# Xinglab/abPOA

Hardware: AMD Instinct MI355X
Metric: read-sets/sec (consensus bit-exact) + DP Gcells/sec (roofline.dp_gcells_per_s) (higher is better)
Workload: dtype int16

## Files before the change

### abpoa_amd/csrc/msa_device.cpp

```cpp
#include <algorithm>
#include <atomic>
#include <chrono>
#include <limits.h>
#include <mutex>
#include <stdio.h>
#include <stdlib.h>
#include <string.h>
#include <thread>
#include <vector>
#include <hip/hip_runtime.h>
#include "engine_options.h"
#include "batch_stream.h"
#include "msa_device.h"
#include "poa_device.h"
#include "poa_graph.h"
#include "dir_plane.h"
#include "msa_batch.h"
#include "msa_device_debug.h"
#include "msa_device_plan.h"

namespace abpoa_hip {

namespace {
#define HIP_OK(expr, code) do { hipError_t e_ = (expr); if (e_ != hipSuccess) { \
// ... 242 lines not shown
    p.nd_base = dg + L.o_base; p.nd_nin = dg + L.o_nin; p.nd_nout = dg + L.o_nout; p.nd_naln = dg + L.o_naln;
    p.nd_in = (int32_t *)(dg + L.o_in); p.nd_out = (int32_t *)(dg + L.o_out); p.nd_outw = (int32_t *)(dg + L.o_outw); p.nd_aln = (int32_t *)(dg + L.o_aln);
    p.nd_inx = (int32_t *)(dg + L.o_inx); p.nd_outx = (int32_t *)(dg + L.o_outx); p.nd_outwx = (int32_t *)(dg + L.o_outwx);
    p.nd_nread = (int32_t *)(dg + L.o_nread); p.nd_row = (int32_t *)(dg + L.o_row);
    p.t_out = (int32_t *)(dg + L.o_tout); p.t_outw = (int32_t *)(dg + L.o_toutw); p.t_in = (int32_t *)(dg + L.o_tin);
    p.nd_rid = (uint64_t *)(dg + L.o_rid); p.msa_rank = (int32_t *)(dg + L.o_mrank); p.msa_off = (const int64_t *)(dg + L.o_msaoff); p.msa_out = nullptr;
    p.row_node[0] = (int32_t *)(dg + L.o_order0); p.row_node[1] = (int32_t *)(dg + L.o_order1);
    p.scratch = (int32_t *)(dr + L.o_scratch);
    p.aln = (AlnDesc *)(dr + L.o_aln_desc); p.out = (AlnOut *)(dr + L.o_out_rec);
    p.row_base = dr + L.o_rbase; p.row_sdist = dr + L.o_rsd; p.row_pd = (uint32_t *)(dr + L.o_rpd); p.row_node_id = (int32_t *)(dr + L.o_rnid);
    p.row_remain = (int32_t *)(dr + L.o_rrem);
    p.pred_off = (int32_t *)(dr + L.o_poff); p.pred_row = (int32_t *)(dr + L.o_pred); p.cigar = (uint64_t *)(dr + L.o_cigar);
    p.out_off = gen_io ? (int32_t *)(dr + L.o_ooff) : nullptr; p.out_row = gen_io ? (int32_t *)(dr + L.o_orow) : nullptr;
    if (pl.amb) {
        p.reads_rc = di + L.o_rc; p.wts_rc = J.any_w ? (int32_t *)(di + L.o_wrc) : nullptr; p.is_rc = dg + L.o_isrc; p.retry = dr + L.o_retry;
        p.out_fwd = (AlnOut *)(dr + L.o_outfwd); p.cigar_fwd = (uint64_t *)(dr + L.o_cigfwd);
    }
    p.cons_node = (int32_t *)(dg + L.o_cnode); p.cons_cov = (int32_t *)(dg + L.o_ccov); p.cons_base = dg + L.o_cbase;
}

int final_lds_plan(const Job &J, DevBatch &b) {
    const DevicePlan &pl = J.pl; const abpoa_hip_scoring_t *sc = &pl.sc;
    int32_t inf_dummy; const int max_bits = abpoa_hip_score_bits(sc, pl.max_node_cap, pl.max_qlen, &inf_dummy); const int pn = max_bits == 16 ? 16 : 8;
    const int64_t width = padded_width(pl.max_qlen, pn);
    const int64_t est_plain = pl.est_cols(width, pl.w_max, pn), est_ragged = std::min<int64_t>(std::max<int64_t>(est_plain, std::min<int64_t>(1024, width)),
            est_plain + pl.max_extra);
    make_lds_plan(sc, pl.max_qlen, max_bits, est_ragged, J.n_sets, &b.lds);
    if (pl.max_extra > 0 && b.lds.fr_cols == 0) make_lds_plan(sc, pl.max_qlen, max_bits, est_plain, J.n_sets, &b.lds);
    if (pl.general) { b.lds.wide_on = 0; b.lds.fr_cols = 0; b.lds.loc_cols = 0; }
    else if (pl.local) {
        b.lds.wide_on = 0;
        if (max_bits != 16 || b.lds.loc_cols <= 0 || (pl.max_qlen / 16 + 1) * 16 > b.lds.loc_cols || pl.max_qlen > b.lds.q_cap) {
                set_err("local alignment outside the device row loop's range"); return ABPOA_HIP_EINVAL; }
    }
    int min_qlen = pl.max_qlen;
    for (int s = 0; s < J.n_sets; ++s) for (int r = 1; r < J.sets[s].n_reads; ++r) min_qlen = std::min(min_qlen, J.sets[s].lens[r]);
    const int min_bits = abpoa_hip_score_bits(sc, 3, min_qlen, &inf_dummy);
    b.bits_mask = (min_bits == 16 ? 1 : 0) | (max_bits == 32 ? 2 : 0);
    const int w_min = std::min(sc->wb + (int)(sc->wf * (float)min_qlen), pl.max_extra ? pl.weff_lo : INT_MAX), w_top = std::max(pl.w_max, pl.weff_hi);
    const bool mixed = pl.max_extra > 0;
    if (!mixed && (w_top < b.lds.wide_w_lo || w_min > b.lds.wide_w_hi)) b.lds.wide_on = 0;
    b.lds.narrow_off = (!mixed && b.lds.wide_on >= 1 && w_min >= b.lds.wide_w_lo && w_top <= b.lds.wide_w_hi) ? 1 : 0;
    return 0;
}

int fill_dev_batch(Job &J, bool *want_general) {
    const DevicePlan &pl = J.pl; Cache &C = *J.C; const Layout &L = J.L; const abpoa_hip_scoring_t *sc = &pl.sc; const PoaDev &p = J.p; DevBatch &b = J.b, &b_rc = J.b_rc;
    uint8_t *di = C.in.dev, *dr = C.rows.dev; const bool gen_io = pl.gen_io(); int rc;
    memset(&b, 0, sizeof(b));
    b.n = J.n_sets; b.m = sc->m;
    if ((rc = final_lds_plan(J, b))) return rc;
    if (!pl.local && !pl.general && (b.lds.fr_cols == 0 || pl.max_qlen > b.lds.q_cap)) { *want_general = true; set_err("band too wide for the fast row loop"); return ABPOA_HIP_EINVAL; }
    b.o1 = sc->gap_open1; b.e1 = sc->gap_ext1; b.o2 = sc->gap_open2; b.e2 = sc->gap_ext2;
    b.align_mode = sc->align_mode; b.gap_mode = sc->gap_mode; b.wb = sc->wb; b.zdrop = sc->zdrop; b.ret_cigar = 1; b.rev_cigar = 0;
    b.want_trace = 0; b.fresh_band = 1; b.want_lr = 0;
    b.dbg = opt_int("ABPOA_HIP_DBG", 0);
    b.mat = (const int32_t *)(di + L.o_mat); b.aln = p.aln; b.out = p.out;
    b.dir_mode = pl.dir ? (pl.dir_wide ? 2 : 1) : 0; b.row_sdist = p.row_sdist; b.row_pd = p.row_pd;
    b.query = p.reads; b.row_base = p.row_base; b.row_node_id = p.row_node_id; b.row_remain = p.row_remain; b.row_active = p.row_base;
    b.pred_off = p.pred_off; b.pred_row = p.pred_row; b.out_off = p.pred_off; b.out_row = p.pred_row;
    b.left = p.scratch; b.right = p.scratch;
    if (gen_io) {
        b.out_off = p.out_off; b.out_row = p.out_row; b.left = (int32_t *)(dr + L.o_left); b.right = (int32_t *)(dr + L.o_right); b.row_active = dr + L.o_act;
    }
    b.dp_beg_sn = (int32_t *)(dr + L.o_bsn); b.dp_end_sn = (int32_t *)(dr + L.o_esn); b.row_cell_off = (int64_t *)(dr + L.o_coff);
    b.row_max_i = (int32_t *)(dr + L.o_rmi);
    b.planes = C.planes.dev; b.cigar = p.cigar;
    b_rc = b;
    if (pl.amb) {
        b.want_lr = (sc->wb >= 0 && !pl.general) ? 1 : 0;
        b_rc = b; b_rc.want_lr = 0; b_rc.fresh_band = sc->wb >= 0 ? 0 : 1;
    }
    return 0;
}

void plan_rounds(Job &J) {
    const DevicePlan &pl = J.pl; const abpoa_hip_scoring_t *sc = &pl.sc; const PoaDev &p = J.p; const DevBatch &b = J.b; DevBatch &b_r = J.b_r;
    bool &dbg_sync = J.dbg_sync, &use_rounds = J.use_rounds; size_t &rounds_lds = J.rounds_lds;
    dbg_sync = opt_on("ABPOA_HIP_DEVSYNC");
    use_rounds = !pl.local && pl.rounds_possible && !dbg_sync && b.lds.wide_on == 0 && !(b.dbg & 64) && pl.max_reads > 2 && !opt_on("ABPOA_HIP_LOCKSTEP");
    b_r = b; rounds_lds = 0;
    if (use_rounds) {
        auto dyn_of = [&](const DevBatch &x) { return std::max<size_t>(std::max<size_t>((size_t)x.lds.total_rows, (size_t)x.lds.total_tail),
                std::max<size_t>((size_t)5 * (size_t)(p.lds_rows > 0 ? p.lds_rows : 0), (size_t)16 * 256)); };
        rounds_lds = dyn_of(b_r);
        int st_lds = 0; int nb = poa_rounds_residency(sc->gap_mode, rounds_lds, &st_lds);
        if (nb < 4 && J.n_sets > nb * 256) {
            const int budget = 160 * 1024 / 4 - st_lds - 512, excess = (int)rounds_lds - budget;
            if (excess > 0 && (size_t)b_r.lds.total_tail == rounds_lds && b_r.lds.bt_bytes_tail - ((excess + 15) & ~15) >= 8 * 1024) {
                b_r.lds.bt_bytes_tail -= (excess + 15) & ~15; b_r.lds.total_tail -= (excess + 15) & ~15;
                rounds_lds = dyn_of(b_r); nb = poa_rounds_residency(sc->gap_mode, rounds_lds, &st_lds);
            }
        }
        b_r.lds.te_on = 0;
        if (b_r.dir_mode && sc->gap_mode != ABPOA_HIP_LINEAR_GAP && !opt_on("ABPOA_HIP_LATE_TAIL")) {
            const int avail = (int)rounds_lds - b_r.lds.phase_off, tables = (SPEC_WK - 1) * SPEC_PM_ROWS * 4;
            const int ring = (b_r.lds.total_rows - b_r.lds.phase_off + 15) & ~15;
            int w_ = ((avail - tables) / SPEC_WK) & ~15, m_ = w_;
            if (w_ < ring) { m_ = ring; w_ = ((avail - tables - m_) / (SPEC_WK - 1)) & ~15; }
            if (w_ >= SPEC_EARLY_MIN) { b_r.lds.te_on = 1; b_r.lds.te_main = m_; b_r.lds.te_w = w_; }
        }
        const int n_cu = device_cu_count(J.device);
        if (nb < 1 || J.n_sets > nb * n_cu) use_rounds = false;
        if (opt_set("ABPOA_HIP_VERBOSE")) fprintf(stderr,
                "[abpoa-hip] all-rounds kernel: %s, %zu B dynamic + %d B static LDS per workgroup, %d workgroups per CU, " "backtrack window %d B, helpers %s (%d + 3 x %d B)\n",
                use_rounds ? "on" : "off", rounds_lds, st_lds, nb, b_r.lds.bt_bytes_tail, b_r.lds.te_on ? "under the row loop" : "after the row loop", b_r.lds.te_main, b_r.lds.te_w);
    }
}

int queue_job(Job &J, DeviceDebug &dbg) {
    const DevicePlan &pl = J.pl; Cache &C = *J.C; const Layout &L = J.L; PoaDev &p = J.p; const DevBatch &b = J.b;
    hipStream_t st = C.stream; uint8_t *hi = C.in.host, *hg = C.graph.host, *dg = C.graph.dev, *dr = C.rows.dev; int rc;
    const int64_t *roff = (const int64_t *)(hi + L.o_roff);
    auto stage = [&](const char *what, int k) { return dbg.stage(what, k); };
    if (pl.gen_io()) HIP_OK(hipMemsetAsync(dr + L.o_act, 1, (size_t)pl.node_tot, st), ABPOA_HIP_ELAUNCH);
    if (pl.amb) HIP_OK(hipMemsetAsync(dg + L.o_isrc, 0, (size_t)pl.tot_reads, st), ABPOA_HIP_ELAUNCH);
    J.t_queue = now_s();
    HIP_OK(hipEventRecord(C.ev[0], st), ABPOA_HIP_ELAUNCH);
    if (stage("upload", 0)) return ABPOA_HIP_ELAUNCH;
    HIP_OK(launch_poa_init(p, st), ABPOA_HIP_ELAUNCH);
    if (stage("init", 0)) return ABPOA_HIP_ELAUNCH;
    dbg.graph_check(0);
    HIP_OK(hipEventRecord(C.ev[1], st), ABPOA_HIP_ELAUNCH);
    for (int k = 1; k < pl.max_reads; ++k) {
        if (k == 2 && !J.rest_up) {
            stage_reads(J, 2, pl.max_reads);
            HIP_OK(hipMemcpyAsync(C.in.dev + L.o_reads + (size_t)J.split_at, hi + L.o_reads + (size_t)J.split_at, (size_t)(roff[pl.tot_reads] - J.split_at),
                    hipMemcpyHostToDevice, C.copy_stream), ABPOA_HIP_ELAUNCH);
            HIP_OK(hipEventRecord(C.ev_copy, C.copy_stream), ABPOA_HIP_ELAUNCH);
            HIP_OK(hipStreamWaitEvent(st, C.ev_copy, 0), ABPOA_HIP_ELAUNCH);
            J.rest_up = true;
        }
        if (J.use_rounds && k == 2) {
            HIP_OK(hipEventRecord(C.ev[2], st), ABPOA_HIP_ELAUNCH);
            HIP_OK(launch_poa_rounds(p, J.b_r, (int32_t *)(dr + L.o_ticket), C.in.host + L.o_rargs, J.slot, 2, J.rounds_lds, st), ABPOA_HIP_ELAUNCH);
            HIP_OK(hipEventRecord(C.ev[3], st), ABPOA_HIP_ELAUNCH);
            break;
        }
        p.round = k;
        hipEvent_t *e = C.ev.data() + 4 * k;
        if (p.order_mode) { HIP_OK(launch_poa_order(p, st), ABPOA_HIP_ELAUNCH); if (stage("row order", k)) return ABPOA_HIP_ELAUNCH; dbg.order_check(k); }
        HIP_OK(launch_poa_prepare(p, st), ABPOA_HIP_ELAUNCH);
        if (stage("prepare", k)) return ABPOA_HIP_ELAUNCH;
        HIP_OK(hipEventRecord(e[0], st), ABPOA_HIP_ELAUNCH);
        if (pl.general) { HIP_OK(launch_dp_general(b, st), ABPOA_HIP_ELAUNCH); HIP_OK(hipEventRecord(e[1], st), ABPOA_HIP_ELAUNCH); }
        else HIP_OK(launch_dp_fast(b, st, e[1]), ABPOA_HIP_ELAUNCH);
        if (stage("dp rows + tail", k)) return ABPOA_HIP_ELAUNCH;
        if (pl.amb) {
            HIP_OK(launch_poa_strand_check(p, st), ABPOA_HIP_ELAUNCH);
            HIP_OK(launch_dp_general(J.b_rc, st), ABPOA_HIP_ELAUNCH);
            HIP_OK(launch_poa_strand_pick(p, st), ABPOA_HIP_ELAUNCH);
            if (stage("strand retry", k)) return ABPOA_HIP_ELAUNCH;
        }
        dbg.balance_report(k, b, e[0], e[1]);
        HIP_OK(hipEventRecord(e[2], st), ABPOA_HIP_ELAUNCH);
        HIP_OK(launch_poa_fuse(p, st), ABPOA_HIP_ELAUNCH);
        if (stage("fuse", k)) return ABPOA_HIP_ELAUNCH;
        dbg.graph_check(k);
        HIP_OK(hipEventRecord(e[3], st), ABPOA_HIP_ELAUNCH);
    }
    if (pl.want_cons) { HIP_OK(launch_poa_consensus(p, st), ABPOA_HIP_ELAUNCH); if (stage("consensus", pl.max_reads)) return ABPOA_HIP_ELAUNCH; }
    if (pl.want_msa) { HIP_OK(launch_poa_msa_rank(p, st), ABPOA_HIP_ELAUNCH); if (stage("msa rank", pl.max_reads)) return ABPOA_HIP_ELAUNCH; }
    HIP_OK(hipMemcpyAsync(hg, dg, J.dl_bytes, hipMemcpyDeviceToHost, st), ABPOA_HIP_ELAUNCH);
    HIP_OK(hipStreamSynchronize(st), ABPOA_HIP_ELAUNCH);
    int64_t msa_total = 0;
    if (pl.want_msa) {
        const PoaState *hs_ = (const PoaState *)(hg + L.o_state);
// ... 173 lines not shown
```

### abpoa_amd/csrc/poa_bodies.h

```cpp
#pragma once
#include <hip/hip_runtime.h>
#include <stdint.h>
#include <limits.h>
#include <string.h>
#include "poa_device.h"
#include "../../include/abpoa_hip.h"

namespace abpoa_hip {

namespace {

__device__ __forceinline__ int imin_(int a, int b) { return a < b ? a : b; }
__device__ __forceinline__ int imax_(int a, int b) { return a > b ? a : b; }
__device__ __forceinline__ int ld_fresh(const int32_t *p) { return __hip_atomic_load(p, __ATOMIC_RELAXED, __HIP_MEMORY_SCOPE_AGENT); }
constexpr int POA_TERM_MAX = 250;
__device__ __forceinline__ int32_t &in_slot(const PoaDev &p, const PoaSet &S, int64_t X, int t) {
    return t < POA_HOT ? p.nd_in[X * POA_HOT + t] : (t < p.in_cap ? p.nd_inx[X * (p.in_cap - POA_HOT) + t - POA_HOT] : p.t_in[S.term0 + t - p.in_cap]);
}
__device__ __forceinline__ int32_t &out_slot(const PoaDev &p, const PoaSet &S, int64_t X, int t) {
    return t < POA_HOT ? p.nd_out[X * POA_HOT + t] : (t < p.out_cap ? p.nd_outx[X * (p.out_cap - POA_HOT) + t - POA_HOT] : p.t_out[S.term0 + t - p.out_cap]);
}
__device__ __forceinline__ int32_t &outw_slot(const PoaDev &p, const PoaSet &S, int64_t X, int t) {
    return t < POA_HOT ? p.nd_outw[X * POA_HOT + t] : (t < p.out_cap ? p.nd_outwx[X * (p.out_cap - POA_HOT) + t - POA_HOT] : p.t_outw[S.term0 + t - p.out_cap]);
}
// ... 162 lines not shown
        const int incl = wave_scan_add(np);
        if (lane == 63) wtot[wave] = incl;
        __syncthreads();
        int before = 0, all = 0;
#pragma unroll
        for (int w_ = 0; w_ < GW; ++w_) { const int x_ = wtot[w_]; all += x_; before += w_ < wave ? x_ : 0; }
        const int off = carry + before + incl - np;
        if (r < n) p.pred_off[N0 + r] = off;
        if (off + np > S.pred_cap) overflow = true;
        carry += all;
        __syncthreads();
    }
    {
        for (int r0 = tid; r0 < n; r0 += 4 * GT) {
            int u[4], np[4], off[4]; int4 i4[4];
#pragma unroll
            for (int j = 0; j < 4; ++j) { const int r = r0 + j * GT; const bool ok = r < n; u[j] = order[ok ? r : 0]; off[j] = p.pred_off[N0 + (ok ? r : 0)];
                                          np[j] = !ok ? 0 : (in_lds ? (int)np_lds[r] : (r > 0 ? (int)p.nd_nin[N0 + u[j]] : 0)); }
#pragma unroll
            for (int j = 0; j < 4; ++j) { if (off[j] + np[j] > S.pred_cap) np[j] = 0; i4[j] = *(const int4 *)(p.nd_in + (N0 + u[j]) * POA_HOT); }
            int pr[4][4];
#pragma unroll
            for (int j = 0; j < 4; ++j) {
                pr[j][0] = np[j] > 0 ? p.nd_row[N0 + i4[j].x] : 0; pr[j][1] = np[j] > 1 ? p.nd_row[N0 + i4[j].y] : 0;
                pr[j][2] = np[j] > 2 ? p.nd_row[N0 + i4[j].z] : 0; pr[j][3] = np[j] > 3 ? p.nd_row[N0 + i4[j].w] : 0;
            }
#pragma unroll
            for (int j = 0; j < 4; ++j) {
                int32_t *dst = p.pred_row + S.pred0 + off[j];
                const int r = r0 + j * GT;
                unsigned long long pdv = ~0ull;
#pragma unroll
                for (int t = 0; t < 4; ++t) {
                    if (t < np[j]) { dst[t] = pr[j][t]; if (r - pr[j][t] <= 254) pdv = (pdv & ~(0xffull << (8 * t))) | ((unsigned long long)(r - pr[j][t]) << (8 * t)); }
                }
                for (int t = POA_HOT; t < np[j]; ++t) { const int pr_ = p.nd_row[N0 + in_slot(p, S, N0 + u[j], t)]; dst[t] = pr_;
                        if (t < 8 && r - pr_ <= 254) pdv = (pdv & ~(0xffull << (8 * t))) | ((unsigned long long)(r - pr_) << (8 * t)); }
                if (r < n) { p.row_pd[2 * (N0 + r)] = (unsigned)pdv; p.row_pd[2 * (N0 + r) + 1] = (unsigned)(pdv >> 32); }
            }
        }
    }
    if (tid == 0) p.pred_off[N0 + n] = carry;
    if (p.out_off) {
        int carry_o = 0;
        for (int t0 = 0; t0 < n; t0 += GT) {
            const int r = t0 + tid;
            const int u = r < n ? order[r] : 0;
            const int no = r < n ? (int)p.nd_nout[N0 + u] : 0;
            const int incl = wave_scan_add(no);
            __syncthreads();
            if (lane == 63) wtot[wave] = incl;
            __syncthreads();
            int before = 0, all = 0;
#pragma unroll
            for (int w_ = 0; w_ < GW; ++w_) { const int x_ = wtot[w_]; all += x_; before += w_ < wave ? x_ : 0; }
            const int off = carry_o + before + incl - no;
            if (r < n) {
                p.out_off[N0 + r] = off;
                if (off + no > S.pred_cap) overflow = true;
                else for (int t = 0; t < no; ++t) p.out_row[S.pred0 + off + t] = p.nd_row[N0 + out_slot(p, S, N0 + u, t)];
            }
            carry_o += all;
        }
        if (tid == 0) p.out_off[N0 + n] = carry_o;
    }
    overflow = __syncthreads_or(overflow);
    if (tid == 0) {
        AlnDesc d; memset(&d, 0, sizeof(d));
        const int qlen = p.read_len[S.read0 + k];
        d.n_rows = n; d.qlen = qlen;
        d.bits = score_bits(p, n, qlen, &d.inf_min);
        d.w = p.wb < 0 ? qlen : p.wb + (int)(p.wf * (float)qlen);
        d.cigar_cap = S.cigar_cap; d.flags = (p.general & 1) ? 0 : ALN_FAST_OK; d.pad0 = S.band_extra;
        d.query_off = p.read_off[S.read0 + k]; d.row0 = N0; d.poff0 = N0; d.pred0 = S.pred0; d.out0 = S.pred0;
        d.plane_off = S.plane_off; d.plane_cap = S.plane_cap / (d.bits / 8); d.cigar_off = S.cigar_off;
        if (overflow || n + qlen + 8 > S.cigar_cap) { st->status = POA_ST_FALLBACK; st->reason = overflow ? POA_WHY_PRED_SLOTS : POA_WHY_CIGAR_SLOTS; d.flags = ALN_SKIP; d.n_rows = 3; }
        p.aln[s] = d;
        p.out[s].status = 0; p.out[s].n_cigar = 0; p.out[s].n_cells = 0;
    }
}

__device__ __forceinline__ void poa_fuse_body(const PoaDev &p, const int s, const int k) {
    const int tid = threadIdx.x, lane = tid & 63, wave = tid >> 6;
    __shared__ int sh_fail, sh_nodes, wtot[GW];
    const PoaSet S = p.sets[s];
    PoaState *st = p.state + s;
    if (uni(st->status) != POA_ST_OK || k >= S.n_reads) return;
    AlnOut res = p.out[s]; res.status = uni(res.status); res.n_cigar = uni(res.n_cigar);
    if (res.status != 0) { if (tid == 0) { st->status = POA_ST_FALLBACK; st->reason = POA_WHY_DP_STATUS + res.status; } return; }
    const int64_t N0 = S.node0;
    const int n_old = uni(st->n_nodes), qlen = p.read_len[S.read0 + k], n_cigar = res.n_cigar;
    const bool rc_read = p.is_rc && uni((int)p.is_rc[S.read0 + k]) != 0;
    const uint8_t *seq = (rc_read ? p.reads_rc : p.reads) + p.read_off[S.read0 + k];
    const uint64_t *cg = p.cigar + S.cigar_off;
    const int cur = uni(st->order_buf);
    const int32_t *order_old = p.row_node[cur] + N0; int32_t *order_new = p.row_node[cur ^ 1] + N0;
    int32_t *cand = p.scratch + S.scratch0, *n_anchor = cand + p.max_qlen, *n_j = n_anchor + p.max_qlen, *addcnt = n_j + p.max_qlen;
    if (p.dig_on) {
        __shared__ unsigned long long sh_dig;
        if (tid == 0) sh_dig = 0;
        __syncthreads();
        unsigned long long part = 0;
        for (int i = tid; i < n_cigar; i += GT) part += poa_cigar_word_mix(cg[i], i);
        if (part) atomicAdd(&sh_dig, part);
        __syncthreads();
        if (tid == 0) st->cigar_dig = poa_cigar_digest_round(st->cigar_dig, k, n_cigar, sh_dig);
    }
    if (n_cigar == 0) return;
    for (int q = tid; q < qlen; q += GT) cand[q] = -1;
    for (int r = tid; r < n_old; r += GT) addcnt[r] = 0;
    __syncthreads();
    for (int i = tid; i < n_cigar; i += GT) {
        const uint64_t w = cg[i];
        if ((int)(w & 0xf) == ABPOA_HIP_CMATCH) cand[(int)((w >> 4) & 0x3fffffff)] = (int)((w >> 34) & 0x3fffffff);
    }
    __syncthreads();
    int n_nodes = n_old, prev_c = 0 , prev_new_c = 0, carry_ar = 0 , carry_sq = -1;
    bool fail = false, fail_slots = false;
    const int32_t *wq = p.wts ? (rc_read ? p.wts_rc : p.wts) + p.read_off[S.read0 + k] : nullptr;
    auto add_edge = [&](bool act, int from, bool from_new, int to, bool to_new, int w) {
        if (!act) return;
        const int64_t F = N0 + from, T = N0 + to;
        int no = from_new ? 0 : (int)p.nd_nout[F];
        int hit = -1;
        if (!from_new && !to_new) for (int t = 0; t < no; ++t) if (out_slot(p, S, F, t) == to) { hit = t; break; }
        if (hit >= 0) outw_slot(p, S, F, hit) += w;
        else {
            const int ni = to_new ? 0 : (int)p.nd_nin[T];
            if (no >= (from == 0 ? imin_(POA_TERM_MAX, p.out_cap + S.n_reads + 2) : p.out_cap) || ni >= (to == 1 ? imin_(POA_TERM_MAX, p.in_cap + S.n_reads + 2) : p.in_cap)) { fail = true;
                    fail_slots = true; return; }
            out_slot(p, S, F, no) = to; outw_slot(p, S, F, no) = w; p.nd_nout[F] = (uint8_t)(no + 1);
            in_slot(p, S, T, ni) = from; p.nd_nin[T] = (uint8_t)(ni + 1);
            hit = no;
            if (hit < p.out_cap) for (int w_ = 0; w_ < p.rid_words; ++w_) p.nd_rid[(F * p.out_cap + hit) * p.rid_words + w_] = 0;
        }
        if (p.rid_words && hit < p.out_cap) p.nd_rid[(F * p.out_cap + hit) * p.rid_words + (k >> 6)] |= 1ull << (k & 63);
        p.nd_nread[F] = (from_new ? 0 : p.nd_nread[F]) + 1;
    };
    __shared__ int sCnt[GW], sMax[GW], sSqm[GW];
    extern __shared__ int fuse_dyn[];
    int *const sNode = fuse_dyn, *const sIsNew = fuse_dyn + GT, *const sAR = fuse_dyn + 2 * GT, *const sSq = fuse_dyn + 3 * GT;
    for (int q0 = 0; q0 < qlen; q0 += GT) {
        const int q = q0 + tid; const bool act = q < qlen;
        const int c = act ? ld_fresh(cand + q) : -1;
        const int b = act ? (int)seq[q] : 0;
        int node = -1; bool isnew = act;
        if (act && c >= 0) {
            if ((int)p.nd_base[N0 + c] == b) { node = c; isnew = false; }
            else {
                const int na = p.nd_naln[N0 + c];
                for (int t = 0; t < na; ++t) { const int a = p.nd_aln[(N0 + c) * p.aln_cap + t]; if ((int)p.nd_base[N0 + a] == b) { node = a; isnew = false; break; } }
            }
        }
        int gv = -1;
        if (act && c >= 0) {
            const int ref = isnew ? c : node;
            gv = p.nd_row[N0 + ref];
            const int na = p.nd_naln[N0 + ref];
            for (int t = 0; t < na; ++t) gv = imax_(gv, p.nd_row[N0 + p.nd_aln[(N0 + ref) * p.aln_cap + t]]);
        }
        const unsigned long long newmask = __ballot(isnew);
        const int rank = __builtin_popcountll(newmask & ((1ull << lane) - 1));
        const int gmax_w = wave_scan_max(gv);
        if (lane == 63) { sCnt[wave] = __builtin_popcountll(newmask); sMax[wave] = gmax_w; }
        __syncthreads();
        int before_cnt = 0, n_new = 0, before_max = carry_ar;
#pragma unroll
        for (int w_ = 0; w_ < GW; ++w_) { const int x_ = sCnt[w_]; n_new += x_; if (w_ < wave) { before_cnt += x_; before_max = imax_(before_max, sMax[w_]); } }
        if (n_nodes + n_new > S.node_cap) { fail = true; break; }
        if (isnew) node = n_nodes + before_cnt + rank;
        if (isnew) {
            const int64_t Y = N0 + node;
            p.nd_base[Y] = (uint8_t)b; p.nd_nin[Y] = 0; p.nd_nout[Y] = 0; p.nd_naln[Y] = 0; p.nd_nread[Y] = 0;
            if (c >= 0) {
                const int na = p.nd_naln[N0 + c];
                if (na + 1 > p.aln_cap) { fail = true; fail_slots = true; }
                else {
                    for (int t = 0; t < na; ++t) {
                        const int other = p.nd_aln[(N0 + c) * p.aln_cap + t];
                        const int no_ = p.nd_naln[N0 + other];
                        p.nd_aln[(N0 + other) * p.aln_cap + no_] = node; p.nd_naln[N0 + other] = (uint8_t)(no_ + 1);
                        p.nd_aln[Y * p.aln_cap + t] = other;
                    }
                    p.nd_aln[(N0 + c) * p.aln_cap + na] = node; p.nd_naln[N0 + c] = (uint8_t)(na + 1);
                    p.nd_aln[Y * p.aln_cap + na] = c; p.nd_naln[Y] = (uint8_t)(na + 1);
                }
            }
        }
        const int AR = imax_(gmax_w, before_max);
        sNode[tid] = node; sIsNew[tid] = (int)isnew; sAR[tid] = AR;
        __syncthreads();
        const int prev = tid > 0 ? sNode[tid - 1] : prev_c, prev_new = tid > 0 ? sIsNew[tid - 1] : prev_new_c, prevAR = tid > 0 ? sAR[tid - 1] : carry_ar;
        add_edge(act, prev, prev_new != 0, node, isnew, (wq && act) ? wq[q] : 1);
        const bool start = isnew && (prev_new == 0 || prevAR != AR);
        const int sq_w = wave_scan_max(start ? q : -1);
        if (lane == 63) sSqm[wave] = sq_w;
        __syncthreads();
        int sq = imax_(sq_w, carry_sq);
#pragma unroll
        for (int w_ = 0; w_ < GW; ++w_) if (w_ < wave) sq = imax_(sq, sSqm[w_]);
        if (isnew) { n_anchor[node - n_old] = AR; n_j[node - n_old] = q - sq + 1; atomicAdd(addcnt + AR, 1); }
        sSq[tid] = sq;
        __syncthreads();
        const int lt = imin_(GT - 1, qlen - 1 - q0);
        prev_c = sNode[lt]; prev_new_c = sIsNew[lt]; carry_ar = sAR[lt]; carry_sq = sSq[lt];
        n_nodes += n_new;
    }
    bool any_fail = __syncthreads_or(fail);
    if (!any_fail) { add_edge(tid == 0, prev_c, prev_new_c != 0, 1, false, wq ? wq[qlen - 1] : 1); any_fail = __syncthreads_or(fail); }
    const bool any_slots = __syncthreads_or(fail_slots);
    if (tid == 0) { sh_fail = any_fail ? (any_slots ? POA_WHY_EDGE_SLOTS : POA_WHY_NODES_IN_FUSE) : POA_WHY_NONE; sh_nodes = n_nodes; }
    __syncthreads();
    if (sh_fail) { if (tid == 0) { st->status = POA_ST_FALLBACK; st->reason = sh_fail; } return; }
    n_nodes = sh_nodes;
    int carry = 0;
    for (int t0 = 0; t0 < n_old; t0 += GT) {
        const int r = t0 + tid;
        const int cnt = r < n_old ? ld_fresh(addcnt + r) : 0;
        const int incl = wave_scan_add(cnt);
        if (lane == 63) wtot[wave] = incl;
        __syncthreads();
        int before = 0, all = 0;
#pragma unroll
        for (int w_ = 0; w_ < GW; ++w_) { const int x_ = wtot[w_]; all += x_; before += w_ < wave ? x_ : 0; }
        const int shift = carry + before + incl - cnt;
        if (r < n_old) { const int u = order_old[r]; order_new[r + shift] = u; p.nd_row[N0 + u] = r + shift; addcnt[r] = shift; }
        carry += all;
        __syncthreads();
    }
    __syncthreads();
    for (int i = tid; i < n_nodes - n_old; i += GT) {
        const int ar = ld_fresh(n_anchor + i), j = ld_fresh(n_j + i);
        const int nr = ar + ld_fresh(addcnt + ar) + j;
        order_new[nr] = n_old + i; p.nd_row[N0 + n_old + i] = nr;
    }
    if (tid == 0) {
        st->n_nodes = n_nodes; st->order_buf = cur ^ 1; st->n_cells += res.n_cells;
        st->algo_bytes += res.n_cells * (p.aln[s].bits / 8) * (p.gap_mode == ABPOA_HIP_AFFINE_GAP ? 5 : 8);
    }
}

}
```

### abpoa_amd/csrc/poa_device.hip

```cpp
#include <algorithm>
#include <map>
#include <mutex>
#include <utility>
#include "poa_bodies.h"

namespace abpoa_hip {

__global__ void __launch_bounds__(64) poa_init_kernel(const PoaDev p) {
    const int s = blockIdx.x, lane = threadIdx.x;
    if (s >= p.n_sets) return;
    const PoaSet S = p.sets[s];
    PoaState *st = p.state + s;
    if (lane == 0) { st->order_buf = 0; st->n_cells = 0; st->algo_bytes = 0; st->reason = POA_WHY_NONE; st->cons_len = 0; st->msa_len = 0; st->cigar_dig = 0; for (int i = 0; i < 4; ++i) st->t_phase[i] = 0;
            st->algo_bytes_before = 0; }
    if (S.n_reads <= 0) { if (lane == 0) { st->n_nodes = 2; st->status = POA_ST_OK; } return; }
    const int L = p.read_len[S.read0];
    const uint8_t *seq = p.reads + p.read_off[S.read0];
    const int n = L + 2;
    if (n > S.node_cap) { if (lane == 0) { st->n_nodes = 2; st->status = POA_ST_FALLBACK; st->reason = POA_WHY_NODES_AT_INIT; } return; }
    const int64_t N0 = S.node0;
    for (int u = lane; u < n; u += 64) {
        const int i = u - 2;
        p.nd_base[N0 + u] = u >= 2 ? seq[i] : 0;
        p.nd_naln[N0 + u] = 0;
// ... 406 lines not shown
            ++msa_rank;
        }
        if (cur == 1) { done = true; break; }
        for (int e0 = 0; e0 < no; e0 += 64) {
            const int e = e0 + lane, key = pops * ORD_KEY + e;
            int v = -1;
            if (e < no) { v = out_slot(p, S, N0 + cur, e); tbl_dec_max<L>(p, g, n, v, key); }
            __syncthreads();
            int total = 0, na = 0;
            if (e < no && tbl_ld<L>(p, g, 0, n, v) == 0) {
                na = p.nd_naln[N0 + v]; bool ready = true;
                for (int t = 0; t < na && ready; ++t) { const int a = p.nd_aln[(N0 + v) * p.aln_cap + t]; ready = tbl_ld<L>(p, g, 0, n, a) == 0 && tbl_ld<L>(p, g, 1, n, a) < key; }
                if (ready) total = 1 + na;
            }
            const int incl = wave_scan_add(total), all = __builtin_amdgcn_readlane(incl, 63);
            if (sp + all > n) return -1;
            if (total) {
                int at = sp + incl - total;
                tbl_st<L>(p, g, 3, n, at, v); tbl_st<L>(p, g, 2, n, v, -1); ++at;
                for (int t = 0; t < na; ++t) { const int a = p.nd_aln[(N0 + v) * p.aln_cap + t]; tbl_st<L>(p, g, 3, n, at, a); tbl_st<L>(p, g, 2, n, a, -1); ++at; }
            }
            sp += all;
            __syncthreads();
        }
        ++pops;
    }
    if (!done) return -1;
    __syncthreads();
    for (int u = lane; u < n; u += 64) {
        int rk = tbl_ld<L>(p, g, 2, n, u); const int na = p.nd_naln[N0 + u];
        for (int t = 0; t < na; ++t) rk = imax_(rk, tbl_ld<L>(p, g, 2, n, p.nd_aln[(N0 + u) * p.aln_cap + t]));
        p.msa_rank[N0 + u] = rk;
    }
    return uni(tbl_ld<L>(p, g, 2, n, 1)) - 1;
}

__global__ void __launch_bounds__(64) poa_msa_rank_kernel(const PoaDev p) {
    const int s = blockIdx.x;
    if (s >= p.n_sets) return;
    const PoaSet S = p.sets[s];
    PoaState *st = p.state + s;
    if (uni(st->status) != POA_ST_OK) return;
    const int n = uni(st->n_nodes);
    if (n <= 2) { if (threadIdx.x == 0) st->msa_len = 0; return; }
    const int len = 4 * n <= 2 * p.order_lds ? poa_msa_rank_body<true>(p, S, n) : poa_msa_rank_body<false>(p, S, n);
    if (threadIdx.x == 0) { if (len < 0) { st->status = POA_ST_FALLBACK; st->reason = POA_WHY_RANK_WALK; st->msa_len = 0; } else st->msa_len = len; }
}

__global__ void __launch_bounds__(GT) poa_msa_fill_kernel(const PoaDev p) {
    const int s = blockIdx.x, tid = threadIdx.x;
    if (s >= p.n_sets) return;
    const PoaSet S = p.sets[s];
    const PoaState *st = p.state + s;
    if (st->status != POA_ST_OK) return;
    const int n = st->n_nodes, len = st->msa_len, rows = S.n_reads + (p.msa_cons ? 1 : 0);
    if (n <= 2 || len <= 0) return;
    uint8_t *out = p.msa_out + p.msa_off[s];
    const int64_t N0 = S.node0, cells = (int64_t)rows * len;
    for (int64_t i = tid; i < cells; i += GT) out[i] = (uint8_t)p.m;
    __syncthreads();
    for (int u = 2 + tid; u < n; u += GT) {
        const int col = p.msa_rank[N0 + u] - 1, no = p.nd_nout[N0 + u]; const uint8_t b = p.nd_base[N0 + u];
        for (int e = 0; e < no; ++e) for (int w_ = 0; w_ < p.rid_words; ++w_) {
            unsigned long long num = p.nd_rid[((N0 + u) * p.out_cap + e) * p.rid_words + w_];
            while (num) { const int r = w_ * 64 + __builtin_ctzll(num); num &= num - 1; if (r < S.n_reads) out[(int64_t)r * len + col] = b; }
        }
    }
    if (p.msa_cons) for (int i = tid; i < st->cons_len; i += GT) out[(int64_t)S.n_reads * len + p.msa_rank[N0 + p.cons_node[S.cons0 + i]] - 1] = p.cons_base[S.cons0 + i];
}

static hipError_t launch_k(void (*kern)(const PoaDev), const PoaDev &p, hipStream_t s) {
    if (p.n_sets <= 0) return hipSuccess;
    hipLaunchKernelGGL(kern, dim3(p.n_sets), dim3(64), 0, s, p);
    return hipGetLastError();
}
hipError_t launch_poa_init(const PoaDev &p, hipStream_t s) { return launch_k(poa_init_kernel, p, s); }
hipError_t launch_poa_prepare(const PoaDev &p, hipStream_t s) {
    if (p.n_sets <= 0) return hipSuccess;
    hipLaunchKernelGGL(poa_prepare_kernel, dim3(p.n_sets), dim3(GT), (size_t)5 * (size_t)(p.lds_rows > 0 ? p.lds_rows : 0), s, p);
    return hipGetLastError();
}
hipError_t launch_poa_fuse(const PoaDev &p, hipStream_t s) {
    if (p.n_sets <= 0) return hipSuccess;
    hipLaunchKernelGGL(poa_fuse_kernel, dim3(p.n_sets), dim3(GT), (size_t)16 * GT, s, p);
    return hipGetLastError();
}
hipError_t launch_poa_strand_check(const PoaDev &p, hipStream_t s) {
    if (p.n_sets <= 0) return hipSuccess;
    hipLaunchKernelGGL(poa_strand_check_kernel, dim3(p.n_sets), dim3(GT), 0, s, p);
    return hipGetLastError();
}
hipError_t launch_poa_strand_pick(const PoaDev &p, hipStream_t s) {
    if (p.n_sets <= 0) return hipSuccess;
    hipLaunchKernelGGL(poa_strand_pick_kernel, dim3(p.n_sets), dim3(GT), 0, s, p);
    return hipGetLastError();
}
hipError_t launch_poa_consensus(const PoaDev &p, hipStream_t s) { return launch_k(poa_consensus_kernel, p, s); }
size_t poa_order_lds_bytes(int node_cap, int ecap) {
    const size_t nc = (size_t)(node_cap > 0 ? node_cap : 0);
    return std::max(4 * (size_t)ORD_RING + 13 * nc + 32, 13 * nc + 2 * (size_t)(ecap > 0 ? ecap : 0) + 64);
}
static hipError_t launch_ord(void (*kern)(const PoaDev), const PoaDev &p, hipStream_t s) {
    if (p.n_sets <= 0) return hipSuccess;
    const size_t lds = poa_order_lds_bytes(p.order_lds, p.order_ecap);
    if (lds > 65536) {
        static std::mutex mu; static std::map<std::pair<const void *, int>, size_t> raised;
        int dev = 0; (void)hipGetDevice(&dev);
        std::lock_guard<std::mutex> lk(mu);
        size_t &have = raised[{(const void *)kern, dev}];
        if (have < lds) { hipError_t e = hipFuncSetAttribute((const void *)kern, hipFuncAttributeMaxDynamicSharedMemorySize, (int)lds); if (e != hipSuccess) return e; have = lds; }
    }
    hipLaunchKernelGGL(kern, dim3(p.n_sets), dim3(64), lds, s, p);
    return hipGetLastError();
}
hipError_t launch_poa_order(const PoaDev &p, hipStream_t s) { return launch_ord(poa_order_kernel, p, s); }
hipError_t launch_poa_msa_rank(const PoaDev &p, hipStream_t s) { return launch_ord(poa_msa_rank_kernel, p, s); }
hipError_t launch_poa_msa_fill(const PoaDev &p, hipStream_t s) {
    if (p.n_sets <= 0) return hipSuccess;
    hipLaunchKernelGGL(poa_msa_fill_kernel, dim3(p.n_sets), dim3(GT), 0, s, p);
    return hipGetLastError();
}

}
```

Measured before the change: 19240.

## Restructure POA fuse body: multi-query per thread, batched loads, shuffle-based carries

```diff
diff --git a/abpoa_amd/csrc/msa_device.cpp b/abpoa_amd/csrc/msa_device.cpp
--- a/abpoa_amd/csrc/msa_device.cpp
+++ b/abpoa_amd/csrc/msa_device.cpp
@@ -348,7 +348,7 @@
     b_r = b; rounds_lds = 0;
     if (use_rounds) {
         auto dyn_of = [&](const DevBatch &x) { return std::max<size_t>(std::max<size_t>((size_t)x.lds.total_rows, (size_t)x.lds.total_tail),
-                std::max<size_t>((size_t)5 * (size_t)(p.lds_rows > 0 ? p.lds_rows : 0), (size_t)16 * 256)); };
+                (size_t)5 * (size_t)(p.lds_rows > 0 ? p.lds_rows : 0)); };
         rounds_lds = dyn_of(b_r);
         int st_lds = 0; int nb = poa_rounds_residency(sc->gap_mode, rounds_lds, &st_lds);
         if (nb < 4 && J.n_sets > nb * 256) {
diff --git a/abpoa_amd/csrc/poa_bodies.h b/abpoa_amd/csrc/poa_bodies.h
--- a/abpoa_amd/csrc/poa_bodies.h
+++ b/abpoa_amd/csrc/poa_bodies.h
@@ -268,7 +268,7 @@
 
 __device__ __forceinline__ void poa_fuse_body(const PoaDev &p, const int s, const int k) {
     const int tid = threadIdx.x, lane = tid & 63, wave = tid >> 6;
-    __shared__ int sh_fail, sh_nodes, wtot[GW];
+    __shared__ int wtot[GW];
     const PoaSet S = p.sets[s];
     PoaState *st = p.state + s;
     if (uni(st->status) != POA_ST_OK || k >= S.n_reads) return;
@@ -304,119 +304,236 @@
     int n_nodes = n_old, prev_c = 0 , prev_new_c = 0, carry_ar = 0 , carry_sq = -1;
     bool fail = false, fail_slots = false;
     const int32_t *wq = p.wts ? (rc_read ? p.wts_rc : p.wts) + p.read_off[S.read0 + k] : nullptr;
-    auto add_edge = [&](bool act, int from, bool from_new, int to, bool to_new, int w) {
-        if (!act) return;
-        const int64_t F = N0 + from, T = N0 + to;
-        int no = from_new ? 0 : (int)p.nd_nout[F];
-        int hit = -1;
-        if (!from_new && !to_new) for (int t = 0; t < no; ++t) if (out_slot(p, S, F, t) == to) { hit = t; break; }
-        if (hit >= 0) outw_slot(p, S, F, hit) += w;
-        else {
-            const int ni = to_new ? 0 : (int)p.nd_nin[T];
-            if (no >= (from == 0 ? imin_(POA_TERM_MAX, p.out_cap + S.n_reads + 2) : p.out_cap) || ni >= (to == 1 ? imin_(POA_TERM_MAX, p.in_cap + S.n_reads + 2) : p.in_cap)) { fail = true;
-                    fail_slots = true; return; }
-            out_slot(p, S, F, no) = to; outw_slot(p, S, F, no) = w; p.nd_nout[F] = (uint8_t)(no + 1);
-            in_slot(p, S, T, ni) = from; p.nd_nin[T] = (uint8_t)(ni + 1);
-            hit = no;
-            if (hit < p.out_cap) for (int w_ = 0; w_ < p.rid_words; ++w_) p.nd_rid[(F * p.out_cap + hit) * p.rid_words + w_] = 0;
-        }
-        if (p.rid_words && hit < p.out_cap) p.nd_rid[(F * p.out_cap + hit) * p.rid_words + (k >> 6)] |= 1ull << (k & 63);
-        p.nd_nread[F] = (from_new ? 0 : p.nd_nread[F]) + 1;
-    };
-    __shared__ int sCnt[GW], sMax[GW], sSqm[GW];
-    extern __shared__ int fuse_dyn[];
-    int *const sNode = fuse_dyn, *const sIsNew = fuse_dyn + GT, *const sAR = fuse_dyn + 2 * GT, *const sSq = fuse_dyn + 3 * GT;
-    for (int q0 = 0; q0 < qlen; q0 += GT) {
-        const int q = q0 + tid; const bool act = q < qlen;
-        const int c = act ? ld_fresh(cand + q) : -1;
-        const int b = act ? (int)seq[q] : 0;
-        int node = -1; bool isnew = act;
-        if (act && c >= 0) {
-            if ((int)p.nd_base[N0 + c] == b) { node = c; isnew = false; }
+    const int out_lim0 = imin_(POA_TERM_MAX, p.out_cap + S.n_reads + 2), in_lim1 = imin_(POA_TERM_MAX, p.in_cap + S.n_reads + 2);
+    constexpr int FP = 4, FA = 3;
+    __shared__ int sCnt[GW], sMax[GW], sSqm[GW], sPrev[2];
+    int *const sLast = wtot;
+    for (int q0 = 0; q0 < qlen; q0 += FP * GT) {
+        const int qb = q0 + FP * tid;
+        bool act[FP]; int c[FP], b[FP], cb[FP], na[FP], gv[FP], am[FP][FA], ab[FP][FA], ar[FP][FA];
+#pragma unroll
+        for (int j = 0; j < FP; ++j) { act[j] = qb + j < qlen; c[j] = act[j] ? ld_fresh(cand + qb + j) : -1; b[j] = act[j] ? (int)seq[qb + j] : 0; }
+        bool any_grp = false;
+#pragma unroll
+        for (int j = 0; j < FP; ++j) {
+            const bool h = c[j] >= 0; const int64_t X = N0 + (h ? c[j] : 0);
+            cb[j] = p.nd_base[X]; na[j] = h ? (int)p.nd_naln[X] : 0; gv[j] = h ? p.nd_row[X] : -1;
+            any_grp |= na[j] > 0;
+        }
+        if (__any(any_grp)) {
+#pragma unroll
+            for (int j = 0; j < FP; ++j)
+#pragma unroll
+                for (int t = 0; t < FA; ++t) { const bool h = t < na[j]; am[j][t] = p.nd_aln[(N0 + (h ? c[j] : 0)) * p.aln_cap + (h ? t : 0)]; }
+#pragma unroll
+            for (int j = 0; j < FP; ++j)
+#pragma unroll
+                for (int t = 0; t < FA; ++t) { const int64_t X = N0 + (t < na[j] ? am[j][t] : 0); ab[j][t] = p.nd_base[X]; ar[j][t] = p.nd_row[X]; }
+        } else {
+#pragma unroll
+            for (int j = 0; j < FP; ++j)
+#pragma unroll
+                for (int t = 0; t < FA; ++t) { am[j][t] = 0; ab[j][t] = 0; ar[j][t] = 0; }
+        }
+        int node[FP]; bool isnew[FP];
+#pragma unroll
+        for (int j = 0; j < FP; ++j) {
+            node[j] = -1; isnew[j] = act[j];
+            if (act[j] && c[j] >= 0) {
+                if (cb[j] == b[j]) { node[j] = c[j]; isnew[j] = false; }
+#pragma unroll
+                for (int t = 0; t < FA; ++t) if (t < na[j]) { if (isnew[j] && ab[j][t] == b[j]) { node[j] = am[j][t]; isnew[j] = false; } gv[j] = imax_(gv[j], ar[j][t]); }
+                for (int t = FA; t < na[j]; ++t) {
+                    const int a = p.nd_aln[(N0 + c[j]) * p.aln_cap + t];
+                    if (isnew[j] && (int)p.nd_base[N0 + a] == b[j]) { node[j] = a; isnew[j] = false; }
+                    gv[j] = imax_(gv[j], p.nd_row[N0 + a]);
+                }
+            }
+        }
+        int cnt = 0, gm = -1;
+#pragma unroll
+        for (int j = 0; j < FP; ++j) { cnt += isnew[j] ? 1 : 0; gm = imax_(gm, gv[j]); }
+        const int icnt = wave_scan_add(cnt), imax = wave_scan_max(gm), lastnode = isnew[FP - 1] ? -1 : node[FP - 1];
+        const int pl = (lane - 1) & 63;
+        const int p_node = shfl(lastnode, pl), p_icnt = shfl(icnt, pl), p_imax = shfl(imax, pl);
+        if (lane == 63) { sCnt[wave] = icnt; sMax[wave] = imax; sLast[wave] = lastnode; }
+        __syncthreads();
+        int before_cnt = 0, n_new = 0, before_max = carry_ar, all_max = carry_ar, wfail = GW;
+#pragma unroll
+        for (int w_ = 0; w_ < GW; ++w_) {
+            const int x_ = sCnt[w_], m_ = sMax[w_];
+            if (w_ < wave) { before_cnt += x_; before_max = imax_(before_max, m_); }
+            n_new += x_; all_max = imax_(all_max, m_);
+            if (wfail == GW && n_nodes + n_new > S.node_cap) wfail = w_;
+        }
+        const bool live = wave < wfail;
+        int AR[FP], pv[FP]; bool pvn[FP], start[FP];
+        int sqt = -1;
+        {
+            const int ex_cnt = lane ? p_icnt : 0;
+            int run = imax_(before_max, lane ? p_imax : -1), id = n_nodes + before_cnt + ex_cnt;
+            int prv = tid == 0 ? prev_c : (lane ? p_node : sLast[wave ? wave - 1 : 0]);
+            bool prvn = tid == 0 ? prev_new_c != 0 : prv < 0;
+            if (tid != 0 && prvn) prv = id - 1;
+#pragma unroll
+            for (int j = 0; j < FP; ++j) {
+                pv[j] = prv; pvn[j] = prvn;
+                const int pAR = run;
+                run = imax_(run, gv[j]); AR[j] = run;
+                if (isnew[j]) node[j] = id++;
+                start[j] = isnew[j] && (!prvn || pAR != run);
+                if (start[j]) sqt = qb + j;
+                prv = node[j]; prvn = isnew[j];
+            }
+        }
+        const int isq = wave_scan_max(sqt), p_isq = shfl(isq, pl);
+        if (lane == 63) sSqm[wave] = isq;
+        {
+            const int qlast = imin_(q0 + FP * GT, qlen) - 1;
+#pragma unroll
+            for (int j = 0; j < FP; ++j) if (qb + j == qlast) { sPrev[0] = node[j]; sPrev[1] = (int)isnew[j]; }
+        }
+#pragma unroll
+        for (int j = 0; j < FP; ++j) if (live && isnew[j]) {
+            const int64_t Y = N0 + node[j], C = N0 + c[j];
+            p.nd_base[Y] = (uint8_t)b[j]; p.nd_nin[Y] = 0; p.nd_nout[Y] = 0; p.nd_naln[Y] = 0; p.nd_nread[Y] = 0;
+            if (c[j] >= 0) {
+                const int na_ = na[j];
+                if (na_ + 1 > p.aln_cap) { fail = true; fail_slots = true; }
+                else {
+#pragma unroll
+                    for (int t = 0; t < FA; ++t) if (t < na_) {
+                        const int other = am[j][t];
+                        p.nd_aln[(N0 + other) * p.aln_cap + na_] = node[j]; p.nd_naln[N0 + other] = (uint8_t)(na_ + 1); p.nd_aln[Y * p.aln_cap + t] = other;
+                    }
+                    for (int t = FA; t < na_; ++t) {
+                        const int other = p.nd_aln[C * p.aln_cap + t];
+                        p.nd_aln[(N0 + other) * p.aln_cap + na_] = node[j]; p.nd_naln[N0 + other] = (uint8_t)(na_ + 1); p.nd_aln[Y * p.aln_cap + t] = other;
+                    }
+                    p.nd_aln[C * p.aln_cap + na_] = node[j]; p.nd_naln[C] = (uint8_t)(na_ + 1);
+                    p.nd_aln[Y * p.aln_cap + na_] = c[j]; p.nd_naln[Y] = (uint8_t)(na_ + 1);
+                }
+            }
+        }
+        bool ea[FP]; int ew[FP], no[FP], ni[FP], nr[FP]; int4 o4[FP];
+#pragma unroll
+        for (int j = 0; j < FP; ++j) {
+            ea[j] = live && act[j];
+            const int64_t F = N0 + ((ea[j] && !pvn[j]) ? pv[j] : 0), T = N0 + ((ea[j] && !isnew[j]) ? node[j] : 0);
+            ew[j] = (wq && act[j]) ? wq[qb + j] : 1;
+            no[j] = p.nd_nout[F]; ni[j] = p.nd_nin[T]; nr[j] = p.nd_nread[F]; o4[j] = *(const int4 *)(p.nd_out + F * POA_HOT);
+        }
+        __syncthreads();
+        int sq = imax_(carry_sq, lane ? p_isq : -1), sq_all = carry_sq;
+#pragma unroll
+        for (int w_ = 0; w_ < GW; ++w_) { const int x_ = sSqm[w_]; sq_all = imax_(sq_all, x_); if (w_ < wave) sq = imax_(sq, x_); }
+#pragma unroll
+        for (int j = 0; j < FP; ++j) {
+            if (start[j]) sq = qb + j;
+            if (live && isnew[j]) { n_anchor[node[j] - n_old] = AR[j]; n_j[node[j] - n_old] = qb + j - sq + 1; atomicAdd(addcnt + AR[j], 1); }
+        }
+        int hit[FP], ow[FP]; int32_t *wp[FP];
+#pragma unroll
+        for (int j = 0; j < FP; ++j) {
+            if (pvn[j]) { no[j] = 0; nr[j] = 0; }
+            if (isnew[j]) ni[j] = 0;
+            hit[j] = -1;
+            if (ea[j] && !pvn[j] && !isnew[j]) {
+                const int to = node[j];
+                if (no[j] > 0 && o4[j].x == to) hit[j] = 0;
+                else if (no[j] > 1 && o4[j].y == to) hit[j] = 1;
+                else if (no[j] > 2 && o4[j].z == to) hit[j] = 2;
+                else if (no[j] > 3 && o4[j].w == to) hit[j] = 3;
+                else for (int t = POA_HOT; t < no[j]; ++t) if (out_slot(p, S, N0 + pv[j], t) == to) { hit[j] = t; break; }
+            }
+            wp[j] = hit[j] >= 0 ? &outw_slot(p, S, N0 + pv[j], hit[j]) : p.nd_outw + N0 * POA_HOT;
+        }
+#pragma unroll
+        for (int j = 0; j < FP; ++j) ow[j] = *wp[j];
+#pragma unroll
+        for (int j = 0; j < FP; ++j) if (ea[j]) {
+            const int from = pv[j], to = node[j];
+            const int64_t F = N0 + from, T = N0 + to;
+            if (hit[j] >= 0) *wp[j] = ow[j] + ew[j];
             else {
-                const int na = p.nd_naln[N0 + c];
-                for (int t = 0; t < na; ++t) { const int a = p.nd_aln[(N0 + c) * p.aln_cap + t]; if ((int)p.nd_base[N0 + a] == b) { node = a; isnew = false; break; } }
-            }
-        }
-        int gv = -1;
-        if (act && c >= 0) {
-            const int ref = isnew ? c : node;
-            gv = p.nd_row[N0 + ref];
-            const int na = p.nd_naln[N0 + ref];
-            for (int t = 0; t < na; ++t) gv = imax_(gv, p.nd_row[N0 + p.nd_aln[(N0 + ref) * p.aln_cap + t]]);
-        }
-        const unsigned long long newmask = __ballot(isnew);
-        const int rank = __builtin_popcountll(newmask & ((1ull << lane) - 1));
-        const int gmax_w = wave_scan_max(gv);
-        if (lane == 63) { sCnt[wave] = __builtin_popcountll(newmask); sMax[wave] = gmax_w; }
-        __syncthreads();
-        int before_cnt = 0, n_new = 0, before_max = carry_ar;
-#pragma unroll
-        for (int w_ = 0; w_ < GW; ++w_) { const int x_ = sCnt[w_]; n_new += x_; if (w_ < wave) { before_cnt += x_; before_max = imax_(before_max, sMax[w_]); } }
-        if (n_nodes + n_new > S.node_cap) { fail = true; break; }
-        if (isnew) node = n_nodes + before_cnt + rank;
-        if (isnew) {
-            const int64_t Y = N0 + node;
-            p.nd_base[Y] = (uint8_t)b; p.nd_nin[Y] = 0; p.nd_nout[Y] = 0; p.nd_naln[Y] = 0; p.nd_nread[Y] = 0;
-            if (c >= 0) {
-                const int na = p.nd_naln[N0 + c];
-                if (na + 1 > p.aln_cap) { fail = true; fail_slots = true; }
-                else {
-                    for (int t = 0; t < na; ++t) {
-                        const int other = p.nd_aln[(N0 + c) * p.aln_cap + t];
-                        const int no_ = p.nd_naln[N0 + other];
-                        p.nd_aln[(N0 + other) * p.aln_cap + no_] = node; p.nd_naln[N0 + other] = (uint8_t)(no_ + 1);
-                        p.nd_aln[Y * p.aln_cap + t] = other;
-                    }
-                    p.nd_aln[(N0 + c) * p.aln_cap + na] = node; p.nd_naln[N0 + c] = (uint8_t)(na + 1);
-                    p.nd_aln[Y * p.aln_cap + na] = c; p.nd_naln[Y] = (uint8_t)(na + 1);
-                }
-            }
-        }
-        const int AR = imax_(gmax_w, before_max);
-        sNode[tid] = node; sIsNew[tid] = (int)isnew; sAR[tid] = AR;
-        __syncthreads();
-        const int prev = tid > 0 ? sNode[tid - 1] : prev_c, prev_new = tid > 0 ? sIsNew[tid - 1] : prev_new_c, prevAR = tid > 0 ? sAR[tid - 1] : carry_ar;
-        add_edge(act, prev, prev_new != 0, node, isnew, (wq && act) ? wq[q] : 1);
-        const bool start = isnew && (prev_new == 0 || prevAR != AR);
-        const int sq_w = wave_scan_max(start ? q : -1);
-        if (lane == 63) sSqm[wave] = sq_w;
-        __syncthreads();
-        int sq = imax_(sq_w, carry_sq);
-#pragma unroll
-        for (int w_ = 0; w_ < GW; ++w_) if (w_ < wave) sq = imax_(sq, sSqm[w_]);
-        if (isnew) { n_anchor[node - n_old] = AR; n_j[node - n_old] = q - sq + 1; atomicAdd(addcnt + AR, 1); }
-        sSq[tid] = sq;
-        __syncthreads();
-        const int lt = imin_(GT - 1, qlen - 1 - q0);
-        prev_c = sNode[lt]; prev_new_c = sIsNew[lt]; carry_ar = sAR[lt]; carry_sq = sSq[lt];
-        n_nodes += n_new;
+                if (no[j] >= (from == 0 ? out_lim0 : p.out_cap) || ni[j] >= (to == 1 ? in_lim1 : p.in_cap)) { fail = true; fail_slots = true; continue; }
+                out_slot(p, S, F, no[j]) = to; outw_slot(p, S, F, no[j]) = ew[j]; p.nd_nout[F] = (uint8_t)(no[j] + 1);
+                in_slot(p, S, T, ni[j]) = from; p.nd_nin[T] = (uint8_t)(ni[j] + 1);
+                hit[j] = no[j];
+                if (hit[j] < p.out_cap) for (int w_ = 0; w_ < p.rid_words; ++w_) p.nd_rid[(F * p.out_cap + hit[j]) * p.rid_words + w_] = 0;
+            }
+            if (p.rid_words && hit[j] < p.out_cap) p.nd_rid[(F * p.out_cap + hit[j]) * p.rid_words + (k >> 6)] |= 1ull << (k & 63);
+            p.nd_nread[F] = nr[j] + 1;
+        }
+        if (wfail < GW) { fail = true; break; }
+        prev_c = sPrev[0]; prev_new_c = sPrev[1]; carry_ar = all_max; carry_sq = sq_all; n_nodes += n_new;
+    }
+    int f3_no = 0, f3_ni = 0, f3_nr = 0; int4 f3_o4 = make_int4(0, 0, 0, 0);
+    if (tid == 0) {
+        const int64_t F = N0 + (prev_new_c ? 0 : prev_c);
+        f3_no = p.nd_nout[F]; f3_ni = p.nd_nin[N0 + 1]; f3_nr = p.nd_nread[F]; f3_o4 = *(const int4 *)(p.nd_out + F * POA_HOT);
     }
     bool any_fail = __syncthreads_or(fail);
-    if (!any_fail) { add_edge(tid == 0, prev_c, prev_new_c != 0, 1, false, wq ? wq[qlen - 1] : 1); any_fail = __syncthreads_or(fail); }
+    if (!any_fail) {
+        if (tid == 0) {
+            const int from = prev_c, w = wq ? wq[qlen - 1] : 1;
+            const bool from_new = prev_new_c != 0;
+            const int64_t F = N0 + from, T = N0 + 1;
+            const int no = from_new ? 0 : f3_no, ni = f3_ni;
+            int hit = -1;
+            if (no > 0 && f3_o4.x == 1) hit = 0;
+            else if (no > 1 && f3_o4.y == 1) hit = 1;
+            else if (no > 2 && f3_o4.z == 1) hit = 2;
+            else if (no > 3 && f3_o4.w == 1) hit = 3;
+            else for (int t = POA_HOT; t < no; ++t) if (out_slot(p, S, F, t) == 1) { hit = t; break; }
+            bool ok = true;
+            if (hit >= 0) outw_slot(p, S, F, hit) += w;
+            else if (no >= (from == 0 ? out_lim0 : p.out_cap) || ni >= in_lim1) { fail = true; fail_slots = true; ok = false; }
+            else {
+                out_slot(p, S, F, no) = 1; outw_slot(p, S, F, no) = w; p.nd_nout[F] = (uint8_t)(no + 1);
+                in_slot(p, S, T, ni) = from; p.nd_nin[T] = (uint8_t)(ni + 1);
+                hit = no;
+                if (hit < p.out_cap) for (int w_ = 0; w_ < p.rid_words; ++w_) p.nd_rid[(F * p.out_cap + hit) * p.rid_words + w_] = 0;
+            }
+            if (ok) {
+                if (p.rid_words && hit < p.out_cap) p.nd_rid[(F * p.out_cap + hit) * p.rid_words + (k >> 6)] |= 1ull << (k & 63);
+                p.nd_nread[F] = (from_new ? 0 : f3_nr) + 1;
+            }
+        }
+        any_fail = __syncthreads_or(fail);
+    }
     const bool any_slots = __syncthreads_or(fail_slots);
-    if (tid == 0) { sh_fail = any_fail ? (any_slots ? POA_WHY_EDGE_SLOTS : POA_WHY_NODES_IN_FUSE) : POA_WHY_NONE; sh_nodes = n_nodes; }
-    __syncthreads();
-    if (sh_fail) { if (tid == 0) { st->status = POA_ST_FALLBACK; st->reason = sh_fail; } return; }
-    n_nodes = sh_nodes;
+    if (any_fail) { if (tid == 0) { st->status = POA_ST_FALLBACK; st->reason = any_slots ? POA_WHY_EDGE_SLOTS : POA_WHY_NODES_IN_FUSE; } return; }
+    constexpr int FR = 8;
+    const int n_add = n_nodes - n_old;
+    int pl_ar = 0, pl_j = 0;
+    if (tid < n_add) { pl_ar = ld_fresh(n_anchor + tid); pl_j = ld_fresh(n_j + tid); }
     int carry = 0;
-    for (int t0 = 0; t0 < n_old; t0 += GT) {
-        const int r = t0 + tid;
-        const int cnt = r < n_old ? ld_fresh(addcnt + r) : 0;
-        const int incl = wave_scan_add(cnt);
+    for (int r0 = 0; r0 < n_old; r0 += FR * GT) {
+        const int rb = r0 + FR * tid;
+        int cn[FR], u[FR], tot = 0;
+#pragma unroll
+        for (int j = 0; j < FR; ++j) { const bool ok = rb + j < n_old; cn[j] = ok ? ld_fresh(addcnt + rb + j) : 0; u[j] = order_old[ok ? rb + j : 0]; }
+#pragma unroll
+        for (int j = 0; j < FR; ++j) tot += cn[j];
+        const int incl = wave_scan_add(tot);
         if (lane == 63) wtot[wave] = incl;
         __syncthreads();
         int before = 0, all = 0;
 #pragma unroll
         for (int w_ = 0; w_ < GW; ++w_) { const int x_ = wtot[w_]; all += x_; before += w_ < wave ? x_ : 0; }
-        const int shift = carry + before + incl - cnt;
-        if (r < n_old) { const int u = order_old[r]; order_new[r + shift] = u; p.nd_row[N0 + u] = r + shift; addcnt[r] = shift; }
+        int shift = carry + before + incl - tot;
+#pragma unroll
+        for (int j = 0; j < FR; ++j) {
+            const int r = rb + j;
+            if (r < n_old) { order_new[r + shift] = u[j]; p.nd_row[N0 + u[j]] = r + shift; addcnt[r] = shift; }
+            shift += cn[j];
+        }
         carry += all;
         __syncthreads();
     }
-    __syncthreads();
-    for (int i = tid; i < n_nodes - n_old; i += GT) {
-        const int ar = ld_fresh(n_anchor + i), j = ld_fresh(n_j + i);
+    for (int i = tid; i < n_add; i += GT) {
+        const int ar = i < GT ? pl_ar : ld_fresh(n_anchor + i), j = i < GT ? pl_j : ld_fresh(n_j + i);
         const int nr = ar + ld_fresh(addcnt + ar) + j;
         order_new[nr] = n_old + i; p.nd_row[N0 + n_old + i] = nr;
     }
diff --git a/abpoa_amd/csrc/poa_device.hip b/abpoa_amd/csrc/poa_device.hip
--- a/abpoa_amd/csrc/poa_device.hip
+++ b/abpoa_amd/csrc/poa_device.hip
@@ -512,7 +512,7 @@
 }
 hipError_t launch_poa_fuse(const PoaDev &p, hipStream_t s) {
     if (p.n_sets <= 0) return hipSuccess;
-    hipLaunchKernelGGL(poa_fuse_kernel, dim3(p.n_sets), dim3(GT), (size_t)16 * GT, s, p);
+    hipLaunchKernelGGL(poa_fuse_kernel, dim3(p.n_sets), dim3(GT), 0, s, p);
     return hipGetLastError();
 }
 hipError_t launch_poa_strand_check(const PoaDev &p, hipStream_t s) {
```

Result: faster. 19610, median of 6 (+1.9%).
